# berkeley-hipie/HIPIE

Measured on AMD Instinct MI355X. Metric: images/sec @1024x1024 ViT-H bs=8 (single-image inference hot path: box, class and mask logits), higher is better.
Workload: dtype f16x3 (split-fp16 operands, fp32 accumulate: fp32-class); 1 GPU; BASELINE.json configs[2]: vit_huge, 1024x1024, batch 8 per GPU, 80 class prompts (L=194), detection; global_batch=8, parallelism=dp1, precision_policy=split, launch=eager

## Files before the change

hipie_amd/csrc/gemm.hip:

```cpp
#include "gemm_tile.h"

namespace hipie {

template <typename T>
__global__ __launch_bounds__(256) void to_hl8_kernel(const T* __restrict__ x, f16_t* __restrict__ out, long rows, int K, long ldx, long ldo,
                                                     float scale) {
  const long gid = (long)blockIdx.x * 256 + threadIdx.x;
  const int gpr = K / 8;
  if (gid >= rows * gpr) return;
  const long r = gid / gpr;
  const int g = (int)(gid - r * gpr);
  const T* src = x + r * ldx + 8 * g;
  f16x8 h, l;
#pragma unroll
  for (int e = 0; e < 8; ++e) {
    f16_t hh, ll;
    hl_split((float)src[e] * scale, hh, ll);
    h[e] = hh;
    l[e] = ll;
  }
  f16_t* dst = out + r * ldo + 16 * g;
  *reinterpret_cast<f16x8*>(dst) = h;
  *reinterpret_cast<f16x8*>(dst + 8) = l;
}


constexpr int kTrRows = 128, kTrCols = 64;
__global__ __launch_bounds__(256) void to_hl8_t_kernel(const float* __restrict__ x, f16_t* __restrict__ out, long rows, int C, long ldx,
                                                       long ldo, long rows_p, float scale) {
  __shared__ float tile[kTrRows][kTrCols + 1];
  const long r0 = (long)blockIdx.x * kTrRows;
  const int c0 = blockIdx.y * kTrCols;
  const int tid = threadIdx.x;
  for (int k = tid; k < kTrRows * (kTrCols / 4); k += 256) {
    const int i = k / (kTrCols / 4), j = (k % (kTrCols / 4)) * 4;
    float v[4] = {0.f, 0.f, 0.f, 0.f};
    if (r0 + i < rows) {
      const float* src = x + (r0 + i) * ldx + c0 + j;
      if (c0 + j + 3 < C && (((uintptr_t)src) & 15) == 0) {
        const float4 q = *reinterpret_cast<const float4*>(src);
        v[0] = q.x; v[1] = q.y; v[2] = q.z; v[3] = q.w;
      } else {
        for (int e = 0; e < 4; ++e) v[e] = c0 + j + e < C ? src[e] : 0.f;
      }
    }
    for (int e = 0; e < 4; ++e) tile[i][j + e] = v[e];
  }
  __syncthreads();
  for (int u = tid; u < kTrCols * (kTrRows / 8); u += 256) {
    const int g = u % (kTrRows / 8), c = u / (kTrRows / 8);
    const long m = r0 + 8 * g;
    if (c0 + c >= C || m >= rows_p) continue;
    f16x8 h, l;
#pragma unroll
    for (int e = 0; e < 8; ++e) {
      f16_t hh, ll;
      hl_split(tile[8 * g + e][c] * scale, hh, ll);
      h[e] = hh;
      l[e] = ll;
    }
    f16_t* dst = out + (long)(c0 + c) * ldo + 2 * m;
    *reinterpret_cast<f16x8*>(dst) = h;
    *reinterpret_cast<f16x8*>(dst + 8) = l;
  }
}

}

using namespace hipie;

namespace hipie {
int launch_gemm_k256(const void* X, long ldx_b, int x_f32, const void* W, long ldw_b, const float* bias, float* out, long ldo, int M, int N,
                     hipStream_t st);
}

static int gemm_impl(const void* A, int64_t lda, const void* W, int64_t ldw, const float* bias, const float* resid, int64_t ldr,
                     void* out, int64_t ldo, const int32_t* out_row, const int32_t* a_row, int64_t a_rows, int M, int N, int K, int in_fmt,
                     int out_fmt, int act, float alpha, float oscale, void* stream) {
  HIPIE_REQUIRE(A && W && out, "gemm: null pointer");
  HIPIE_REQUIRE(in_fmt == HIPIE_F16 || in_fmt == HIPIE_HL8 || in_fmt == HIPIE_F32, "gemm: operand format %d (HIPIE_F16 | HIPIE_HL8 | HIPIE_F32)",
                in_fmt);
  HIPIE_REQUIRE(out_fmt == HIPIE_F32 || out_fmt == HIPIE_F16 || out_fmt == HIPIE_HL8, "gemm: output format %d", out_fmt);
  HIPIE_REQUIRE(act >= 0 && act <= 3, "gemm: activation %d (0 none, 1 gelu, 2 relu, 3 quick-gelu)", act);
  HIPIE_REQUIRE(M > 0 && N > 0 && K > 0 && N % 8 == 0, "gemm: M=%d N=%d K=%d (N must be a multiple of 8)", M, N, K);
  const bool a_f32 = in_fmt == HIPIE_F32;
  const bool split = in_fmt == HIPIE_HL8 || a_f32;
  if (a_f32) lda *= 2;
  const int kq = split ? 32 : 64;
  HIPIE_REQUIRE(K % kq == 0, "gemm: K=%d must be a multiple of %d", K, kq);
  const int epr = split ? 2 * K : K;
  HIPIE_TRY(gm_check_operands("gemm", lda, ldw, epr, 320));
  HIPIE_TRY(gm_check_out("gemm", ldo, out_fmt, N));
  HIPIE_TRY(gm_check_resid("gemm", resid, ldr, N));
  HIPIE_TRY(gm_check_aligned("gemm", {A, W, out, bias, resid}));
  GemmParams p;
  gm_set_operands(p, A, lda, W, ldw, M, N, K, kq);
  p.bias = bias; p.resid = resid; p.ldr = ldr; p.out = (char*)out; p.ldo = ldo; p.out_row = out_row; p.a_row = a_row;
  p.out_fmt = out_fmt; p.act = act; p.alpha = alpha; p.oscale = oscale;
  hipStream_t st = (hipStream_t)stream;
  static const int k256_mode = [] { const char* e = study_env("HIPIE_GEMM_K256"); return e ? atoi(e) : 2; }();
  const bool k256_on = k256_mode == 1 || (k256_mode == 2 && N >= 384);
  if (k256_on && split && K == 256 && out_fmt == HIPIE_F32 && act == 0 && resid == nullptr && out_row == nullptr && a_row == nullptr &&
      alpha == 1.f && oscale == 1.f && N % 32 == 0 && M >= 8192 && ldw * 2 == 1024 && (long)M * p.lda_b < (1L << 32))
    return launch_gemm_k256(A, p.lda_b, a_f32 ? 1 : 0, W, p.ldw_b, bias, (float*)out, ldo, M, N, st);
  const bool wide = (N % 320 == 0);
  static const int small_on = [] { const char* e = study_env("HIPIE_GEMM_SMALL"); return e ? atoi(e) : 1; }();
  static const long small_tiles = [] { const char* e = study_env("HIPIE_GEMM_SMALL_MAXTILES"); return e ? atol(e) : 96L; }();
  const bool small_ok = small_on && (long)((M + 255) / 256) * ((N + (wide ? 319 : 255)) / (wide ? 320 : 256)) < small_tiles;
#ifdef HIPIE_GEMM_VARIANTS
  { const char* e = study_env("HIPIE_GEMM_VARIANT"); const int v = e ? atoi(e) : 0;
    if (split && wide && v == 1) return launch_gemm<320, true, 1>(p, st);
    if (split && wide && v == 3) return launch_gemm<320, true, 3>(p, st); }
  { const char* e = study_env("HIPIE_GEMM_VARIANT"); if (e) p.variant = atoi(e); }
  p.prio_mode = gemm2_prio();
  if (split && gemm2_mode() == 4) {
    const bool w160 = (N % 160 == 0);
    if (a_f32) return w160 ? launch_gemm4<5, 2>(p, st) : launch_gemm4<4, 2>(p, st);
    return w160 ? launch_gemm4<5, 0>(p, st) : launch_gemm4<4, 0>(p, st);
  }
  if (split && gemm2_mode() == 2) {
    const bool w160 = (N % 160 == 0);
    if (a_f32) return w160 ? launch_gemm3<5, 2>(p, st) : launch_gemm3<4, 2>(p, st);
    return w160 ? launch_gemm3<5, 0>(p, st) : launch_gemm3<4, 0>(p, st);
  }
  if (split && gemm2_mode() == 1) {
    const bool w160 = (N % 160 == 0);
    if (a_f32) return w160 ? launch_gemm2<5, 2>(p, st) : launch_gemm2<4, 2>(p, st);
    return w160 ? launch_gemm2<5, 0>(p, st) : launch_gemm2<4, 0>(p, st);
  }
#endif
  if (split && small_ok && a_row == nullptr) return a_f32 ? launch_gemm_small<2>(p, st) : launch_gemm_small<0>(p, st);
  if (a_f32) return wide ? launch_gemm<320, true, 2>(p, st) : launch_gemm<256, true, 2>(p, st);
  if (split) return wide ? launch_gemm<320, true>(p, st) : launch_gemm<256, true>(p, st);
  return wide ? launch_gemm<320, false>(p, st) : launch_gemm<256, false>(p, st);
}

extern "C" int hipie_gemm(const void* A, int64_t lda, const void* W, int64_t ldw, const float* bias, const float* resid, int64_t ldr,
                          void* out, int64_t ldo, const int32_t* out_row, int M, int N, int K, int in_fmt, int out_fmt, int act, float alpha,
                          float oscale, void* stream) {
  return gemm_impl(A, lda, W, ldw, bias, resid, ldr, out, ldo, out_row, nullptr, 0, M, N, K, in_fmt, out_fmt, act, alpha, oscale, stream);
}

extern "C" int hipie_gemm_gather(const void* A, int64_t lda, int64_t a_rows, const int32_t* a_row, const void* W, int64_t ldw, const float* bias,
                                 const float* resid, int64_t ldr, void* out, int64_t ldo, const int32_t* out_row, int M, int N, int K, int in_fmt,
                                 int out_fmt, int act, float alpha, float oscale, void* stream) {
  HIPIE_REQUIRE(a_row != nullptr && a_rows > 0, "gemm_gather: a_row map / operand row count missing");
  HIPIE_REQUIRE(in_fmt == HIPIE_HL8 || in_fmt == HIPIE_F32, "gemm_gather: split operands only (HIPIE_HL8 | HIPIE_F32 rows)");
  HIPIE_REQUIRE((long)a_rows * lda * (in_fmt == HIPIE_F32 ? 4 : 2) < (1L << 32), "gemm_gather: the gathered operand must stay below 4 GiB");
  return gemm_impl(A, lda, W, ldw, bias, resid, ldr, out, ldo, out_row, a_row, a_rows, M, N, K, in_fmt, out_fmt, act, alpha, oscale, stream);
}

extern "C" int hipie_gemm_batched(const void* A, int64_t lda, int64_t a_outer, int64_t a_inner, const void* W, int64_t ldw, int64_t w_outer,
                                  int64_t w_inner, void* out, int64_t ldo, int64_t o_outer, int64_t o_inner, int n_outer, int n_inner, int M,
                                  int N, int K, int out_fmt, float alpha, void* stream) {
  HIPIE_REQUIRE(A && W && out, "gemm_batched: null pointer");
  HIPIE_REQUIRE(out_fmt == HIPIE_F32 || out_fmt == HIPIE_HL8, "gemm_batched: output format %d (HIPIE_F32 | HIPIE_HL8)", out_fmt);
  HIPIE_REQUIRE(M > 0 && N > 0 && K > 0 && N % 8 == 0 && K % 32 == 0, "gemm_batched: M=%d N=%d K=%d (N %% 8, K %% 32)", M, N, K);
  HIPIE_TRY(gm_check_batch_shape("gemm_batched", n_outer, n_inner));
  HIPIE_TRY(gm_check_operands("gemm_batched", lda, ldw, 2 * K, 320));
  HIPIE_TRY(gm_check_out("gemm_batched", ldo, out_fmt, N));
  HIPIE_TRY(gm_check_batch_offsets("gemm_batched", a_outer, a_inner, w_outer, w_inner, o_outer, o_inner));
  HIPIE_TRY(gm_check_aligned("gemm_batched", {A, W, out}));
  GemmParams p;
  gm_set_operands(p, A, lda, W, ldw, M, N, K);
  gm_set_batch(p, n_inner, a_outer, a_inner, w_outer, w_inner, o_outer, o_inner, out_fmt == HIPIE_F32 ? 4 : 2);
  p.out = (char*)out; p.ldo = ldo; p.out_fmt = out_fmt; p.alpha = alpha;
  hipStream_t st = (hipStream_t)stream;
  const int batches = n_outer * n_inner;
#ifdef HIPIE_GEMM_VARIANTS
  if (gemm2_mode() == 1) return (N % 160 == 0) ? launch_gemm2<5, 0>(p, st, batches) : launch_gemm2<4, 0>(p, st, batches);
#endif
  return (N % 320 == 0) ? launch_gemm<320, true>(p, st, batches) : launch_gemm<256, true>(p, st, batches);
}

extern "C" int hipie_gemm_batched_resid(const void* A, int64_t lda, int64_t a_outer, int64_t a_inner, const void* W, int64_t ldw, int64_t w_outer,
                                        int64_t w_inner, const float* bias, const float* resid, int64_t ldr, int64_t r_outer, int64_t r_inner,
                                        float* out, int64_t ldo, int64_t o_outer, int64_t o_inner, int n_outer, int n_inner, int M, int N, int K,
                                        float alpha, void* stream) {
  HIPIE_REQUIRE(A && W && out, "gemm_batched_resid: null pointer");
  HIPIE_REQUIRE(M > 0 && N > 0 && K > 0 && N % 8 == 0 && K % 32 == 0, "gemm_batched_resid: M=%d N=%d K=%d (N %% 8, K %% 32)", M, N, K);
  HIPIE_TRY(gm_check_batch_shape("gemm_batched_resid", n_outer, n_inner));
  HIPIE_TRY(gm_check_operands("gemm_batched_resid", lda, ldw, 2 * K, 320));
  HIPIE_TRY(gm_check_out("gemm_batched_resid", ldo, HIPIE_F32, N));
  HIPIE_REQUIRE(resid == nullptr || (ldr >= N && ldr % 4 == 0 && ((r_outer | r_inner) % 4) == 0), "gemm_batched_resid: residual strides %ld / %ld / %ld",
                (long)ldr, (long)r_outer, (long)r_inner);
  HIPIE_TRY(gm_check_batch_offsets("gemm_batched_resid", a_outer, a_inner, w_outer, w_inner, o_outer, o_inner));
  HIPIE_TRY(gm_check_aligned("gemm_batched_resid", {A, W, out, bias, resid}));
  GemmParams p;
  gm_set_operands(p, A, lda, W, ldw, M, N, K);
  gm_set_batch(p, n_inner, a_outer, a_inner, w_outer, w_inner, o_outer, o_inner, 4);
  p.out = (char*)out; p.ldo = ldo; p.alpha = alpha;
  p.bias = bias; p.resid = resid; p.ldr = ldr; p.r_bo = r_outer; p.r_bi = r_inner;
  return (N % 320 == 0) ? launch_gemm<320, true>(p, (hipStream_t)stream, n_outer * n_inner) : launch_gemm<256, true>(p, (hipStream_t)stream, n_outer * n_inner);
}

extern "C" int hipie_gemm_batched_softmax(const void* A, int64_t lda, int64_t a_outer, int64_t a_inner, const void* W, int64_t ldw, int64_t w_outer,
                                          int64_t w_inner, void* out, int64_t ldo, int64_t o_outer, int64_t o_inner, int n_outer, int n_inner,
                                          int M, int N, int K, const unsigned char* mask, int L, float clamp, float alpha, void* stream) {
  HIPIE_REQUIRE(A && W && out, "gemm_batched_softmax: null pointer");
  HIPIE_REQUIRE(M > 0 && N > 0 && N <= 256 && N % 8 == 0 && K > 0 && K % 32 == 0 && L > 0 && L <= N,
                "gemm_batched_softmax: M=%d N=%d K=%d L=%d (N <= 256: the row must fit one column tile)", M, N, K, L);
  HIPIE_TRY(gm_check_batch_shape("gemm_batched_softmax", n_outer, n_inner));
  HIPIE_TRY(gm_check_operands("gemm_batched_softmax", lda, ldw, 2 * K, 320));
  HIPIE_TRY(gm_check_out("gemm_batched_softmax", ldo, HIPIE_HL8, N));
  HIPIE_TRY(gm_check_batch_offsets("gemm_batched_softmax", a_outer, a_inner, w_outer, w_inner, o_outer, o_inner));
  HIPIE_TRY(gm_check_aligned("gemm_batched_softmax", {A, W, out}));
  GemmParams p;
  gm_set_operands(p, A, lda, W, ldw, M, N, K);
  gm_set_batch(p, n_inner, a_outer, a_inner, w_outer, w_inner, o_outer, o_inner, 2);
  p.out = (char*)out; p.ldo = ldo; p.out_fmt = HIPIE_HL8; p.alpha = alpha;
  p.softmax = 1; p.sm_L = L; p.sm_clamp = clamp; p.sm_mask = mask;
  return launch_gemm<256, true>(p, (hipStream_t)stream, n_outer * n_inner);
}

extern "C" int hipie_conv3x3_split(const void* x, int64_t ldx, const void* w, const float* bias, void* out, int64_t ldo, int64_t rows, int Wp,
                                   int C, int N, int in_fmt, int out_fmt, int act, void* stream) {
  HIPIE_REQUIRE(x && w && out, "conv3x3_split: null pointer");
  HIPIE_REQUIRE(in_fmt == HIPIE_HL8 || in_fmt == HIPIE_F32, "conv3x3_split: input format %d (HIPIE_HL8 | HIPIE_F32 rows)", in_fmt);
  HIPIE_REQUIRE(out_fmt == HIPIE_F32 || out_fmt == HIPIE_HL8, "conv3x3_split: output format %d (HIPIE_F32 | HIPIE_HL8)", out_fmt);
  HIPIE_REQUIRE(act >= 0 && act <= 2, "conv3x3_split: activation %d", act);
  HIPIE_REQUIRE(rows > 0 && rows < (1L << 31) && Wp >= 3 && C > 0 && C % 32 == 0 && N > 0 && N % 8 == 0, "conv3x3_split: rows=%ld Wp=%d C=%d N=%d",
                (long)rows, Wp, C, N);
  if (in_fmt == HIPIE_F32) ldx *= 2;
  HIPIE_REQUIRE(ldx >= 2 * C && ldx % 8 == 0, "conv3x3_split: input row stride %ld", (long)ldx);
  HIPIE_REQUIRE((long)(256 + Wp + 2) * ldx * 2 < (1L << 31), "conv3x3_split: row stride too large");
  HIPIE_TRY(gm_check_out("conv3x3_split", ldo, out_fmt, N));
  HIPIE_TRY(gm_check_aligned("conv3x3_split", {x, w, out, bias}));
  GemmParams p;
  gm_set_operands(p, x, ldx, w, (long)2 * 9 * C, (int)rows, N, 9 * C);
  p.bias = bias; p.out = (char*)out; p.ldo = ldo; p.out_fmt = out_fmt; p.act = act;
  p.conv_kpt = C / 32; p.conv_wp = Wp;
  hipStream_t st = (hipStream_t)stream;
  const bool wide = (N % 320 == 0);
  if (in_fmt == HIPIE_F32) return wide ? launch_gemm<320, true, 2>(p, st) : launch_gemm<256, true, 2>(p, st);
  return wide ? launch_gemm<320, true>(p, st) : launch_gemm<256, true>(p, st);
}

extern "C" int hipie_to_hl8(const void* x, int64_t ldx, void* out, int64_t ldo, int64_t rows, int K, int x_dtype, float scale, void* stream) {
  HIPIE_REQUIRE(x && out && rows > 0 && K > 0 && K % 8 == 0, "to_hl8: rows=%ld K=%d (K must be a multiple of 8)", (long)rows, K);
  HIPIE_REQUIRE(ldx >= K && ldo >= 2 * K && ldo % 8 == 0, "to_hl8: row strides %ld / %ld", (long)ldx, (long)ldo);
  const long n = rows * (K / 8);
  const dim3 grid((unsigned)((n + 255) / 256));
  hipStream_t st = (hipStream_t)stream;
  switch (x_dtype) {
    case HIPIE_F32: hipLaunchKernelGGL(to_hl8_kernel<float>, grid, dim3(256), 0, st, (const float*)x, (f16_t*)out, rows, K, ldx, ldo, scale); break;
    case HIPIE_F16: hipLaunchKernelGGL(to_hl8_kernel<f16_t>, grid, dim3(256), 0, st, (const f16_t*)x, (f16_t*)out, rows, K, ldx, ldo, scale); break;
    default: return set_err(HIPIE_EINVAL, "to_hl8: dtype %d", x_dtype);
  }
  return check_launch("to_hl8");
}

extern "C" int hipie_to_hl8_t(const void* x, int64_t ldx, void* out, int64_t ldo, int64_t rows, int C, int64_t rows_p, float scale, void* stream) {
  HIPIE_REQUIRE(x && out && rows > 0 && C > 0, "to_hl8_t: rows=%ld C=%d", (long)rows, C);
  HIPIE_REQUIRE(rows_p >= rows && rows_p % 8 == 0 && ldx >= C && ldo >= 2 * rows_p && ldo % 8 == 0, "to_hl8_t: rows_p=%ld (>= rows, multiple of 8), strides %ld / %ld",
                (long)rows_p, (long)ldx, (long)ldo);
  HIPIE_REQUIRE(((uintptr_t)out % 16) == 0, "to_hl8_t: output must be 16-byte aligned");
  const long tiles_r = (rows_p + kTrRows - 1) / kTrRows, tiles_c = (C + kTrCols - 1) / kTrCols;
  HIPIE_REQUIRE(tiles_c <= 65535, "to_hl8_t: C=%d too wide", C);
  hipLaunchKernelGGL(to_hl8_t_kernel, dim3((unsigned)tiles_r, (unsigned)tiles_c), dim3(256), 0, (hipStream_t)stream, (const float*)x, (f16_t*)out,
                     (long)rows, C, (long)ldx, (long)ldo, (long)rows_p, scale);
  return check_launch("to_hl8_t");
}
```

hipie_amd/csrc/gemm_tile.h:

```cpp
#pragma once
#include <stdlib.h>

#include <initializer_list>

#include "common.h"
#include "gelu.h"
#include "mfma.h"
#include "wave.h"

namespace hipie {

struct GemmParams {
  const char* A = nullptr; const char* W = nullptr; const float* bias = nullptr; const float* resid = nullptr; char* out = nullptr;
  const int32_t* out_row = nullptr;
  const int32_t* a_row = nullptr;
  long lda_b = 0, ldw_b = 0;
  long ldr = 0, ldo = 0;
  int M = 0, N = 0, K = 0;
  int nkt = 0;
  int tiles_m = 0, tiles_n = 0;
  int group_m = 0;
  int out_fmt = HIPIE_F32, act = 0;
  float alpha = 1.f, oscale = 1.f;
  int nbi = 1;
  long a_bo = 0, a_bi = 0, w_bo = 0, w_bi = 0, o_bo = 0, o_bi = 0;
  int conv_kpt = 0, conv_wp = 0;
  int softmax = 0, sm_L = 0;
  float sm_clamp = 0.f;
  const unsigned char* sm_mask = nullptr;
  const float* sm_bias = nullptr;
  long r_bo = 0, r_bi = 0;
  const float* ln_g = nullptr; const float* ln_b = nullptr; float ln_eps = 0.f;
  char* out2 = nullptr; long ldo2 = 0;
  int variant = 0;
  int prio_mode = 0;
};

__device__ __forceinline__ unsigned int gm_pack2(float a, float b) {
  typedef _Float16 h2 __attribute__((ext_vector_type(2)));
  h2 v;
  v[0] = (f16_t)a;
  v[1] = (f16_t)b;
  return __builtin_bit_cast(unsigned int, v);
}

__device__ __forceinline__ unsigned int gm_pack2h(f16_t a, f16_t b) {
  typedef _Float16 h2 __attribute__((ext_vector_type(2)));
  h2 v;
  v[0] = a;
  v[1] = b;
  return __builtin_bit_cast(unsigned int, v);
}


typedef _Float16 gm_h2 __attribute__((ext_vector_type(2)));
__device__ __forceinline__ void gm_split2(float x0, float x1, unsigned int& H, unsigned int& L) {
  x0 = __builtin_amdgcn_fmed3f(x0, -65504.f, 65504.f);
  x1 = __builtin_amdgcn_fmed3f(x1, -65504.f, 65504.f);
  hl_split2(x0, x1, H, L);
}

template <int NG>
__device__ __forceinline__ void gm_epi_vals(const float (&x)[NG][4], const int G0, const float4* rq, const float* sb, const long m, const bool mok,
                                            const int nb, const int hi, const GemmParams& p, const bool has_res) {
  typedef unsigned int u32x2 __attribute__((ext_vector_type(2)));
  typedef unsigned int u32x4 __attribute__((ext_vector_type(4)));
  const float alpha = p.alpha, osc = p.oscale;
  const int act = p.act, ofmt = p.out_fmt;
  float v[NG][4];
#pragma unroll
  for (int g = 0; g < NG; ++g) {
    const float4 b4 = *reinterpret_cast<const float4*>(sb + 8 * (G0 + g) + 4 * hi);
    v[g][0] = x[g][0] * alpha + b4.x;
    v[g][1] = x[g][1] * alpha + b4.y;
    v[g][2] = x[g][2] * alpha + b4.z;
    v[g][3] = x[g][3] * alpha + b4.w;
  }
  if (act == 1) {
#pragma unroll
    for (int g = 0; g < NG; ++g)
#pragma unroll
      for (int e = 0; e < 4; ++e) v[g][e] = gm_gelu(v[g][e]);
  } else if (act == 2) {
#pragma unroll
    for (int g = 0; g < NG; ++g)
#pragma unroll
      for (int e = 0; e < 4; ++e) v[g][e] = fmaxf(v[g][e], 0.f);
  } else if (act == 3) {
#pragma unroll
    for (int g = 0; g < NG; ++g)
#pragma unroll
      for (int e = 0; e < 4; ++e) v[g][e] = v[g][e] / (1.f + expf(-1.702f * v[g][e]));
  }
  if (has_res) {
#pragma unroll
    for (int g = 0; g < NG; ++g) { v[g][0] += rq[g].x; v[g][1] += rq[g].y; v[g][2] += rq[g].z; v[g][3] += rq[g].w; }
  }
  if (osc != 1.f) {
#pragma unroll
    for (int g = 0; g < NG; ++g)
#pragma unroll
      for (int e = 0; e < 4; ++e) v[g][e] *= osc;
  }
  if (ofmt == HIPIE_F16) {
#pragma unroll
    for (int g = 0; g < NG; g += 2) {
      const u32x2 s0 = __builtin_amdgcn_permlane32_swap(gm_pack2(v[g][0], v[g][1]), gm_pack2(v[g + 1][0], v[g + 1][1]), false, false);
      const u32x2 s1 = __builtin_amdgcn_permlane32_swap(gm_pack2(v[g][2], v[g][3]), gm_pack2(v[g + 1][2], v[g + 1][3]), false, false);
      const int n = nb + 8 * (G0 + g + hi);
      if (mok && n < p.N) *reinterpret_cast<u32x4*>(reinterpret_cast<f16_t*>(p.out) + m * p.ldo + n) = (u32x4){s0[0], s1[0], s0[1], s1[1]};
    }
  } else {
    u32x4 piece[NG];
    if (ofmt == HIPIE_F32) {
#pragma unroll
      for (int g = 0; g < NG; ++g)
        piece[g] = (u32x4){__builtin_bit_cast(unsigned int, v[g][0]), __builtin_bit_cast(unsigned int, v[g][1]),
                           __builtin_bit_cast(unsigned int, v[g][2]), __builtin_bit_cast(unsigned int, v[g][3])};
    } else {
#pragma unroll
      for (int g = 0; g < NG; ++g) {
        unsigned int H0, L0, H1, L1;
        gm_split2(v[g][0], v[g][1], H0, L0);
        gm_split2(v[g][2], v[g][3], H1, L1);
#if defined(__HIP_DEVICE_COMPILE__) && !defined(HIPIE_NO_FMA_MIX)
        asm volatile("s_nop 1" : "+v"(H0), "+v"(L0), "+v"(H1), "+v"(L1));
#endif
        const u32x2 s0 = __builtin_amdgcn_permlane32_swap(H0, L0, false, false);
        const u32x2 s1 = __builtin_amdgcn_permlane32_swap(H1, L1, false, false);
        piece[g] = (u32x4){s0[0], s1[0], s0[1], s1[1]};
      }
    }
    const long rowb = (m * p.ldo) * (ofmt == HIPIE_F32 ? 4 : 2) + (long)nb * 4 + 16 * hi;
#pragma unroll
    for (int g = 0; g < NG; ++g)
      if (mok && nb + 8 * (G0 + g) < p.N) *reinterpret_cast<u32x4*>(p.out + rowb + 32 * (G0 + g)) = piece[g];
  }
}

template <int G0, int NG>
__device__ __forceinline__ void gm_epi_quads(const f32x16& a, const float4* rq, const float* sb, const long m, const bool mok, const int nb,
                                             const int hi, const GemmParams& p, const bool has_res) {
  float x[NG][4];
#pragma unroll
  for (int g = 0; g < NG; ++g)
#pragma unroll
    for (int e = 0; e < 4; ++e) x[g][e] = a[4 * (G0 + g) + e];
  gm_epi_vals<NG>(x, G0, rq, sb, m, mok, nb, hi, p, has_res);
}

template <int BN, bool SPLIT, int VAR>
__global__ __launch_bounds__(512, 2) void gemm_kernel(const GemmParams pin) {
  GemmParams p = pin;
  int vtile = -1;
  if (VAR == 8) {
    const int nblk = p.tiles_m * p.tiles_n * p.nbi;
    const int id = blockIdx.x, xcd = id & 7, j = id >> 3;
    const int q = nblk >> 3, r = nblk & 7;
    const int v = (xcd < r ? xcd * (q + 1) : r * (q + 1) + (xcd - r) * q) + j;
    const int bo = blockIdx.y, bi = v % p.nbi;
    vtile = v / p.nbi;
    p.A += bo * p.a_bo + bi * p.a_bi;
    p.W += bo * p.w_bo + bi * p.w_bi;
    p.out += bo * p.o_bo + bi * p.o_bi;
    if (p.sm_mask != nullptr) p.sm_mask += (long)bo * p.sm_L;
    if (p.sm_bias != nullptr) p.sm_bias += ((long)bo * p.nbi + bi) * p.N;
  } else if (gridDim.y > 1) {
    const int bo = blockIdx.y / p.nbi, bi = blockIdx.y - bo * p.nbi;
    p.A += bo * p.a_bo + bi * p.a_bi;
    p.W += bo * p.w_bo + bi * p.w_bi;
    p.out += bo * p.o_bo + bi * p.o_bi;
    if (p.sm_mask != nullptr) p.sm_mask += (long)bo * p.sm_L;
    if (p.sm_bias != nullptr) p.sm_bias += (long)blockIdx.y * p.N;
    if (p.resid != nullptr) p.resid += bo * p.r_bo + bi * p.r_bi;
  }
  constexpr int BM = 256;
  constexpr int ROWS = BM + BN;
  constexpr int STAGE = ROWS * 128;
  constexpr int NI = ROWS / 64;
  constexpr int NJ = BN / 64;
  constexpr int KS = SPLIT ? 2 : 4;
  constexpr int SUB = KS * NJ;
  constexpr bool AF32 = VAR == 2 || VAR == 6;
  constexpr bool LNE = VAR == 4 || VAR == 6;
  typedef Mfma32<f16_t>::frag frag;

  extern __shared__ __attribute__((aligned(128))) char smem[];

  const int tid = threadIdx.x, lane = tid & 63;
  const int wave = __builtin_amdgcn_readfirstlane(tid >> 6);
  const int wm = wave & 3, wn = wave >> 2;
  const int li = lane & 31, hi = lane >> 5;

  int tm, tn;
  {
    const int nblk = p.tiles_m * p.tiles_n;
    const int id = blockIdx.x, xcd = id & 7, j = id >> 3;
    const int q = nblk >> 3, r = nblk & 7;
    const int v = (VAR == 8) ? vtile : (xcd < r ? xcd * (q + 1) : r * (q + 1) + (xcd - r) * q) + j;
    if (p.group_m > 1) {
      const int gsz = p.group_m * p.tiles_n;
      const int g = v / gsz, w = v - g * gsz;
      const int rows = min(p.group_m, p.tiles_m - g * p.group_m);
      tn = w / rows;
      tm = g * p.group_m + (w - tn * rows);
    } else {
      tm = v / p.tiles_n;
      tn = v - tm * p.tiles_n;
    }
  }
  const int m0 = tm * BM, n0 = tn * BN;

  unsigned int dvoff[NI];
  {
    const int rl = lane >> 3, cp = lane & 7;
#pragma unroll
    for (int i = 0; i < NI; ++i) {
      const int r = 8 * (8 * i + wave) + rl;
      const int c = cp ^ ((r >> 1) & 7);
      if (r < BM) {
        const int mr = min(r, p.M - 1 - m0);
        dvoff[i] = p.a_row != nullptr ? (unsigned int)((long)p.a_row[m0 + mr] * p.lda_b + 16 * c) : (unsigned int)((long)mr * p.lda_b + 16 * c);
      } else dvoff[i] = (unsigned int)((long)min(r - BM, p.N - 1 - n0) * p.ldw_b + 16 * c);
    }
  }
  const char* abase = p.a_row != nullptr ? p.A : p.A + (long)m0 * p.lda_b;
  const char* wbase = p.W + (long)n0 * p.ldw_b;
  const unsigned int lds0 = (unsigned int)reinterpret_cast<uintptr_t>((__attribute__((address_space(3))) char*)smem);

  auto dma = [&](const int i, const int kt, const int stage) {
    const bool isa = (8 * (8 * i + wave)) < BM;
    long ko = (long)kt * 128;
    if (isa && p.conv_kpt) {
      const int tap = kt / p.conv_kpt, r = kt - tap * p.conv_kpt, dy = tap / 3;
      ko = ((long)(dy - 1) * p.conv_wp + (tap - 3 * dy - 1)) * p.lda_b + (long)r * 128;
    }
    const char* sb = (isa ? abase : wbase) + ko;
    dma16(sb, dvoff[i], __builtin_amdgcn_readfirstlane(lds0 + (unsigned int)(stage * STAGE + 1024 * (8 * i + wave))));
  };

  const int swz = (li >> 1) & 7;
  const char* xrow = smem + (wm * 64 + li) * 128;
  const char* wrow = smem + (BM + wn * (BN / 2) + li) * 128;
  auto choff = [&](const int ks, const int lo) -> int { return 16 * ((SPLIT ? (2 * (2 * ks + hi) + lo) : (2 * ks + hi)) ^ swz); };

  f32x16 acc[NJ][2];
#pragma unroll
  for (int j = 0; j < NJ; ++j)
#pragma unroll
    for (int t = 0; t < 2; ++t)
#pragma unroll
      for (int r = 0; r < 16; ++r) acc[j][t][r] = 0.f;

#ifdef HIPIE_GEMM_VARIANTS
  const int nkt = (VAR == 3) ? 0 : p.nkt;
  if (VAR != 3)
#else
  const int nkt = p.nkt;
#endif
  {
#pragma unroll
    for (int i = 0; i < NI; ++i) dma(i, 0, 0);
  }
  __builtin_amdgcn_s_waitcnt(vmcnt(0));
  __syncthreads();

  for (int kt = 0; kt < nkt; ++kt) {
    const int st = kt & 1;
    const bool more = kt + 1 < nkt;
    const char* xs = xrow + st * STAGE;
    const char* ws = wrow + st * STAGE;
    frag xa[2][2][2];
    frag wa[2][2];
    auto load_x = [&](const int ks) {
#pragma unroll
      for (int t = 0; t < 2; ++t) {
        xa[ks & 1][0][t] = *reinterpret_cast<const frag*>(xs + t * 4096 + choff(ks, 0));
        if (SPLIT) xa[ks & 1][1][t] = *reinterpret_cast<const frag*>(xs + t * 4096 + choff(ks, 1));
      }
    };
    auto load_w = [&](const int s) {
      const int ks = s / NJ, j = s % NJ;
      wa[s & 1][0] = *reinterpret_cast<const frag*>(ws + j * 4096 + choff(ks, 0));
      if (SPLIT) wa[s & 1][1] = *reinterpret_cast<const frag*>(ws + j * 4096 + choff(ks, 1));
    };
    load_x(0);
    load_w(0);
    constexpr int DMA_BY = SPLIT ? 4 : 6;
    constexpr int PER = (NI + DMA_BY - 1) / DMA_BY;
    frag cx[2][2];
#pragma unroll
    for (int s = 0; s < SUB; ++s) {
      const int ks = s / NJ, j = s % NJ;
      if (s + 1 < SUB) {
        if ((s + 1) % NJ == 0) load_x(ks + 1);
        load_w(s + 1);
      }
      if (AF32 && j == 0) {
#pragma unroll
        for (int t = 0; t < 2; ++t) {
          const f32x4 a = __builtin_bit_cast(f32x4, xa[ks & 1][0][t]), b = __builtin_bit_cast(f32x4, xa[ks & 1][1][t]);
#pragma unroll
          for (int e = 0; e < 4; ++e) {
            f16_t hh, ll;
            hl_split(a[e], hh, ll);
            cx[0][t][e] = hh; cx[1][t][e] = ll;
            hl_split(b[e], hh, ll);
            cx[0][t][4 + e] = hh; cx[1][t][4 + e] = ll;
          }
        }
      }
      const frag wh = wa[s & 1][0];
      const frag xh0 = AF32 ? cx[0][0] : xa[ks & 1][0][0], xh1 = AF32 ? cx[0][1] : xa[ks & 1][0][1];
      if (SPLIT) {
        const frag wl = wa[s & 1][1];
        const frag xl0 = AF32 ? cx[1][0] : xa[ks & 1][1][0], xl1 = AF32 ? cx[1][1] : xa[ks & 1][1][1];
        acc[j][0] = Mfma32<f16_t>::mma(wl, xh0, acc[j][0]);
        acc[j][1] = Mfma32<f16_t>::mma(wl, xh1, acc[j][1]);
        acc[j][0] = Mfma32<f16_t>::mma(wh, xl0, acc[j][0]);
        acc[j][1] = Mfma32<f16_t>::mma(wh, xl1, acc[j][1]);
      }
      acc[j][0] = Mfma32<f16_t>::mma(wh, xh0, acc[j][0]);
      acc[j][1] = Mfma32<f16_t>::mma(wh, xh1, acc[j][1]);
      if (more) {
#pragma unroll
        for (int i = s * PER; i < (s + 1) * PER && i < NI; ++i) dma(i, kt + 1, st ^ 1);
      }
    }
    __builtin_amdgcn_s_waitcnt(vmcnt(0));
    __syncthreads();
  }

  bool has_res = p.resid != nullptr;
#ifdef HIPIE_GEMM_VARIANTS
  if (VAR == 1 && p.alpha != 12345.f) return;
#endif
  const int act = p.act, ofmt = p.out_fmt;
  const float alpha = p.alpha, osc = p.oscale;
  float* sbias = reinterpret_cast<float*>(smem);
  if (tid < BN) sbias[tid] = (p.bias != nullptr && n0 + tid < p.N) ? p.bias[n0 + tid] : 0.f;
  if (SPLIT && LNE && BN == 256) {
    float* lg = sbias + 256;
    float* lb = lg + 256;
    float* red = lb + 256;
    if (tid < 256) { lg[tid] = p.ln_g[tid]; lb[tid] = p.ln_b[tid]; }
    __syncthreads();
    float su[2] = {0.f, 0.f};
    f32x4 rr[2][4];
    auto ln_res = [&](const int blk, f32x4 (&dst)[4]) {
      const int t = blk / NJ, j = blk % NJ;
      const int m = min(m0 + wm * 64 + t * 32 + li, p.M - 1);
#pragma unroll
      for (int g = 0; g < 4; ++g) {
        const int n = wn * (BN / 2) + j * 32 + 8 * g + 4 * hi;
        dst[g] = *reinterpret_cast<const f32x4*>(p.resid + (long)m * p.ldr + n);
      }
    };
    ln_res(0, rr[0]);
#pragma unroll
    for (int blk = 0; blk < 2 * NJ; ++blk) {
      const int t = blk / NJ, j = blk % NJ;
      if (blk + 1 < 2 * NJ) ln_res(blk + 1, rr[(blk + 1) & 1]);
#pragma unroll
      for (int g = 0; g < 4; ++g) {
        const int n = wn * (BN / 2) + j * 32 + 8 * g + 4 * hi;
        const f32x4 b4 = *reinterpret_cast<const f32x4*>(sbias + n);
#pragma unroll
        for (int e = 0; e < 4; ++e) {
          float x = acc[j][t][4 * g + e] * p.alpha + b4[e];
          x += rr[blk & 1][g][e];
          acc[j][t][4 * g + e] = x;
          su[t] += x;
        }
      }
#if defined(__HIP_DEVICE_COMPILE__)
      __builtin_amdgcn_sched_barrier(0);
#endif
    }
#pragma unroll
    for (int t = 0; t < 2; ++t) {
      su[t] += __shfl_xor(su[t], 32);
      if (hi == 0) red[wn * 256 + wm * 64 + t * 32 + li] = su[t];
    }
    __syncthreads();
    float mean[2], sq[2];
#pragma unroll
    for (int t = 0; t < 2; ++t) {
      mean[t] = (su[t] + red[(wn ^ 1) * 256 + wm * 64 + t * 32 + li]) / 256.f;
      float q = 0.f;
#pragma unroll
      for (int j = 0; j < NJ; ++j)
#pragma unroll
        for (int r = 0; r < 16; ++r) { const float d = acc[j][t][r] - mean[t]; q += d * d; }
      sq[t] = q + __shfl_xor(q, 32);
    }
    __syncthreads();
#pragma unroll
    for (int t = 0; t < 2; ++t)
      if (hi == 0) red[wn * 256 + wm * 64 + t * 32 + li] = sq[t];
    __syncthreads();
    float rstd[2];
#pragma unroll
    for (int t = 0; t < 2; ++t) rstd[t] = rsqrtf((sq[t] + red[(wn ^ 1) * 256 + wm * 64 + t * 32 + li]) / 256.f + p.ln_eps);
#pragma unroll
    for (int j = 0; j < NJ; ++j) {
#pragma unroll
      for (int t = 0; t < 2; ++t)
#pragma unroll
        for (int g = 0; g < 4; ++g) {
          const int n = wn * (BN / 2) + j * 32 + 8 * g + 4 * hi;
          const f32x4 g4 = *reinterpret_cast<const f32x4*>(lg + n), b4 = *reinterpret_cast<const f32x4*>(lb + n);
#pragma unroll
          for (int e = 0; e < 4; ++e) acc[j][t][4 * g + e] = (acc[j][t][4 * g + e] - mean[t]) * rstd[t] * g4[e] + b4[e];
        }
#if defined(__HIP_DEVICE_COMPILE__)
      __builtin_amdgcn_sched_barrier(0);
#endif
    }
    __syncthreads();
    if (tid < BN) sbias[tid] = 0.f;
    p.alpha = 1.f; p.act = 0; p.oscale = 1.f; p.out_fmt = HIPIE_F32;
    has_res = false;
  }
  if (SPLIT && (VAR == 0 || VAR == 8) && BN == 256 && p.softmax) {
    float* kb = sbias + 256;
    float* red = kb + 256;
    float* cb = red + 512;
    if (tid < 256) kb[tid] = (tid < p.sm_L && (p.sm_mask == nullptr || p.sm_mask[tid] != 0)) ? 0.f : -INFINITY;
    if (VAR == 8 && tid < 256) cb[tid] = (p.sm_bias != nullptr && tid < p.N) ? p.sm_bias[tid] : 0.f;
    __syncthreads();
    const float cl = p.sm_clamp;
    float mx[2] = {-INFINITY, -INFINITY};
#pragma unroll
    for (int t = 0; t < 2; ++t)
#pragma unroll
      for (int j = 0; j < NJ; ++j)
#pragma unroll
        for (int g = 0; g < 4; ++g) {
          const f32x4 k4 = *reinterpret_cast<const f32x4*>(kb + wn * (BN / 2) + j * 32 + 8 * g + 4 * hi);
          f32x4 c4 = {0.f, 0.f, 0.f, 0.f};
          if (VAR == 8) c4 = *reinterpret_cast<const f32x4*>(cb + wn * (BN / 2) + j * 32 + 8 * g + 4 * hi);
#pragma unroll
          for (int e = 0; e < 4; ++e) {
            float x = acc[j][t][4 * g + e] * p.alpha;
            if (VAR == 8) x += c4[e];
            if (cl > 0.f) x = __builtin_amdgcn_fmed3f(x, -cl, cl);
            x += k4[e];
            acc[j][t][4 * g + e] = x;
            mx[t] = fmaxf(mx[t], x);
          }
        }
#pragma unroll
    for (int t = 0; t < 2; ++t) {
      mx[t] = fmaxf(mx[t], __shfl_xor(mx[t], 32));
      if (hi == 0) red[wn * 256 + wm * 64 + t * 32 + li] = mx[t];
    }
    __syncthreads();
    float sm[2];
#pragma unroll
    for (int t = 0; t < 2; ++t) {
      const float m = fmaxf(mx[t], red[(wn ^ 1) * 256 + wm * 64 + t * 32 + li]);
      const float m2 = (m == -INFINITY) ? 0.f : m * 1.4426950408889634f;
      float su = 0.f;
#pragma unroll
      for (int j = 0; j < NJ; ++j)
#pragma unroll
        for (int r = 0; r < 16; ++r) {
          const float pv = __builtin_amdgcn_exp2f(acc[j][t][r] * 1.4426950408889634f - m2);
          acc[j][t][r] = pv;
          su += pv;
        }
      sm[t] = su + __shfl_xor(su, 32);
    }
    __syncthreads();
#pragma unroll
    for (int t = 0; t < 2; ++t)
      if (hi == 0) red[wn * 256 + wm * 64 + t * 32 + li] = sm[t];
    __syncthreads();
#pragma unroll
    for (int t = 0; t < 2; ++t) {
      const float tot = sm[t] + red[(wn ^ 1) * 256 + wm * 64 + t * 32 + li];
      const float inv = tot > 0.f ? 1.f / tot : 0.f;
#pragma unroll
      for (int j = 0; j < NJ; ++j)
#pragma unroll
        for (int r = 0; r < 16; ++r) acc[j][t][r] *= inv;
    }
    p.alpha = 1.f;
  }
  __syncthreads();
  float4 rq[2][4];
  long orow[2];
#pragma unroll
  for (int t = 0; t < 2; ++t) {
    const int m = m0 + wm * 64 + t * 32 + li;
    orow[t] = (m < p.M) ? (p.out_row != nullptr ? (long)p.out_row[m] : (long)m) : -1;
  }
  auto load_res = [&](const int t, const int j, float4 (&dst)[4]) {
#pragma unroll
    for (int g = 0; g < 4; ++g) {
      const int n = n0 + wn * (BN / 2) + j * 32 + 8 * g + 4 * hi;
      dst[g] = (has_res && orow[t] >= 0 && n < p.N) ? *reinterpret_cast<const float4*>(p.resid + orow[t] * p.ldr + n) : make_float4(0.f, 0.f, 0.f, 0.f);
    }
  };
  const int passes = (LNE && p.out2 != nullptr) ? 2 : 1;
#pragma unroll
  for (int pass = 0; pass < 2; ++pass) {
    if (pass >= passes) break;
    if (pass == 1) { p.out = p.out2; p.ldo = p.ldo2; p.out_fmt = HIPIE_HL8; }
    load_res(0, 0, rq[0]);
#pragma unroll
    for (int t = 0; t < 2; ++t) {
      const long m = orow[t];
      const bool mok = m >= 0;
#pragma unroll
      for (int j = 0; j < NJ; ++j) {
        const int blk = t * NJ + j;
        if (blk + 1 < 2 * NJ) load_res((blk + 1) / NJ, (blk + 1) % NJ, rq[(blk + 1) & 1]);
        const int nb = n0 + wn * (BN / 2) + j * 32;
        gm_epi_quads<0, 4>(acc[j][t], rq[blk & 1], sbias + (nb - n0), m, mok, nb, hi, p, has_res);
#if defined(__HIP_DEVICE_COMPILE__)
        if (LNE) __builtin_amdgcn_sched_barrier(0);
#endif
      }
    }
  }
}



template <int VAR>
__global__ __launch_bounds__(256, 2) void gemm_small_kernel(const GemmParams p) {
  constexpr int BM = 64, BN = 128, ROWS = BM + BN, STAGE = ROWS * 128, NI = ROWS / 32;
  typedef Mfma32<f16_t>::frag frag;
  extern __shared__ __attribute__((aligned(128))) char smem[];

  const int tid = threadIdx.x, lane = tid & 63;
  const int wave = __builtin_amdgcn_readfirstlane(tid >> 6);
  const int li = lane & 31, hi = lane >> 5;
  const int tm = blockIdx.x / p.tiles_n, tn = blockIdx.x - tm * p.tiles_n;
  const int m0 = tm * BM, n0 = tn * BN;

  unsigned int dvoff[NI];
  {
    const int rl = lane >> 3, cp = lane & 7;
#pragma unroll
    for (int i = 0; i < NI; ++i) {
      const int r = 8 * (4 * i + wave) + rl;
      const int c = cp ^ ((r >> 1) & 7);
      if (r < BM) dvoff[i] = (unsigned int)((long)min(r, p.M - 1 - m0) * p.lda_b + 16 * c);
      else dvoff[i] = (unsigned int)((long)min(r - BM, p.N - 1 - n0) * p.ldw_b + 16 * c);
    }
  }
  const char* abase = p.A + (long)m0 * p.lda_b;
  const char* wbase = p.W + (long)n0 * p.ldw_b;
  const unsigned int lds0 = (unsigned int)reinterpret_cast<uintptr_t>((__attribute__((address_space(3))) char*)smem);
  auto dma_stage = [&](const int kt, const int slot) {
#pragma unroll
    for (int i = 0; i < NI; ++i) {
      const bool isa = (8 * (4 * i + wave)) < BM;
      dma16((isa ? abase : wbase) + (long)kt * 128, dvoff[i],
               __builtin_amdgcn_readfirstlane(lds0 + (unsigned int)(slot * STAGE + 1024 * (4 * i + wave))));
    }
  };

  const int swz = (li >> 1) & 7;
  const char* xrow = smem + li * 128;
  const char* wrow = smem + (BM + wave * 32 + li) * 128;
  auto choff = [&](const int ks, const int lo) -> int { return 16 * ((2 * (2 * ks + hi) + lo) ^ swz); };

  f32x16 acc[2];
#pragma unroll
  for (int t = 0; t < 2; ++t)
#pragma unroll
    for (int r = 0; r < 16; ++r) acc[t][r] = 0.f;

  const int nkt = p.nkt;
  dma_stage(0, 0);
  if (nkt > 1) dma_stage(1, 1);
  int slot = 0;
  for (int kt = 0; kt < nkt; ++kt) {
    if (kt + 1 < nkt) __builtin_amdgcn_s_waitcnt(vmcnt(NI));
    else __builtin_amdgcn_s_waitcnt(vmcnt(0));
    __syncthreads();
    if (kt + 2 < nkt) dma_stage(kt + 2, slot == 0 ? 2 : slot - 1);
    const char* xs = xrow + slot * STAGE;
    const char* ws = wrow + slot * STAGE;
#pragma unroll
    for (int ks = 0; ks < 2; ++ks) {
      frag xh[2], xl[2];
#pragma unroll
      for (int t = 0; t < 2; ++t) {
        xh[t] = *reinterpret_cast<const frag*>(xs + t * 4096 + choff(ks, 0));
        xl[t] = *reinterpret_cast<const frag*>(xs + t * 4096 + choff(ks, 1));
      }
      const frag wh = *reinterpret_cast<const frag*>(ws + choff(ks, 0));
      const frag wl = *reinterpret_cast<const frag*>(ws + choff(ks, 1));
      if (VAR == 2) {
#pragma unroll
        for (int t = 0; t < 2; ++t) {
          const f32x4 a = __builtin_bit_cast(f32x4, xh[t]), b = __builtin_bit_cast(f32x4, xl[t]);
#pragma unroll
          for (int e = 0; e < 4; ++e) {
            f16_t hh, ll;
            hl_split(a[e], hh, ll);
            xh[t][e] = hh; xl[t][e] = ll;
            hl_split(b[e], hh, ll);
            xh[t][4 + e] = hh; xl[t][4 + e] = ll;
          }
        }
      }
#pragma unroll
      for (int t = 0; t < 2; ++t) {
        acc[t] = Mfma32<f16_t>::mma(wl, xh[t], acc[t]);
        acc[t] = Mfma32<f16_t>::mma(wh, xl[t], acc[t]);
        acc[t] = Mfma32<f16_t>::mma(wh, xh[t], acc[t]);
      }
    }
    slot = slot == 2 ? 0 : slot + 1;
  }

  const bool has_res = p.resid != nullptr;
  __syncthreads();
  float* sbias = reinterpret_cast<float*>(smem);
  if (tid < BN) sbias[tid] = (p.bias != nullptr && n0 + tid < p.N) ? p.bias[n0 + tid] : 0.f;
  __syncthreads();
  const int nb = n0 + wave * 32;
#pragma unroll
  for (int t = 0; t < 2; ++t) {
    const int mm = m0 + t * 32 + li;
    const long m = (mm < p.M) ? (p.out_row != nullptr ? (long)p.out_row[mm] : (long)mm) : -1;
    float4 rq[4];
#pragma unroll
    for (int g = 0; g < 4; ++g) {
      const int n = nb + 8 * g + 4 * hi;
      rq[g] = (has_res && m >= 0 && n < p.N) ? *reinterpret_cast<const float4*>(p.resid + m * p.ldr + n) : make_float4(0.f, 0.f, 0.f, 0.f);
    }
    gm_epi_quads<0, 4>(acc[t], rq, sbias + wave * 32, m, m >= 0, nb, hi, p, has_res);
  }
}

template <int VAR>
static int launch_gemm_small(GemmParams& p, hipStream_t st) {
  constexpr size_t lds = (size_t)3 * (64 + 128) * 128;
  p.tiles_m = (p.M + 63) / 64;
  p.tiles_n = (p.N + 127) / 128;
  auto kern = gemm_small_kernel<VAR>;
  static LdsLimit limit;
  limit.raise((const void*)kern, lds);
  hipLaunchKernelGGL(kern, dim3((unsigned)(p.tiles_m * p.tiles_n)), dim3(256), lds, st, p);
  return check_launch("gemm_small");
}

#ifdef HIPIE_GEMM_VARIANTS
#include "../../tools/ubench/gemm_overlap_study.h"
#endif

template <int BN, bool SPLIT, int VAR = 0>
static int launch_gemm(GemmParams& p, hipStream_t st, int batches = 1) {
  constexpr size_t lds = (size_t)2 * (256 + BN) * 128;
  p.tiles_m = (p.M + 255) / 256;
  p.tiles_n = (p.N + BN - 1) / BN;
  p.group_m = p.tiles_n > 4 ? 8 : 0;
  auto kern = gemm_kernel<BN, SPLIT, VAR>;
  static LdsLimit limit;
  limit.raise((const void*)kern, lds);
  if (VAR == 8)
    hipLaunchKernelGGL(kern, dim3((unsigned)(p.tiles_m * p.tiles_n * p.nbi), (unsigned)(batches / p.nbi)), dim3(512), lds, st, p);
  else
    hipLaunchKernelGGL(kern, dim3((unsigned)(p.tiles_m * p.tiles_n), (unsigned)batches), dim3(512), lds, st, p);
  return check_launch("gemm");
}

static inline void gm_set_operands(GemmParams& p, const void* A, long lda, const void* W, long ldw, int M, int N, int K, int kq = 32) {
  p.A = (const char*)A; p.W = (const char*)W;
  p.lda_b = lda * 2; p.ldw_b = ldw * 2;
  p.M = M; p.N = N; p.K = K; p.nkt = K / kq;
}

static inline void gm_set_batch(GemmParams& p, int n_inner, long a_outer, long a_inner, long w_outer, long w_inner, long o_outer, long o_inner,
                                long osz) {
  p.nbi = n_inner;
  p.a_bo = a_outer * 2; p.a_bi = a_inner * 2; p.w_bo = w_outer * 2; p.w_bi = w_inner * 2; p.o_bo = o_outer * osz; p.o_bi = o_inner * osz;
}

static inline int gm_check_operands(const char* who, long lda, long ldw, int epr, int bn) {
  if (!(lda >= epr && ldw >= epr && lda % 8 == 0 && ldw % 8 == 0))
    return set_err(HIPIE_EINVAL, "%s: operand row strides %ld / %ld (>= %d, multiples of 8)", who, lda, ldw, epr);
  if (!(256 * lda * 2 < (1L << 31) && bn * ldw * 2 < (1L << 31))) return set_err(HIPIE_EINVAL, "%s: row stride too large", who);
  return 0;
}

static inline int gm_check_out(const char* who, long ldo, int out_fmt, int N) {
  const int opr = out_fmt == HIPIE_HL8 ? 2 * N : N;
  if (!(ldo >= opr && ldo % 4 == 0)) return set_err(HIPIE_EINVAL, "%s: output row stride %ld (>= %d)", who, ldo, opr);
  return 0;
}

static inline int gm_check_resid(const char* who, const float* resid, long ldr, int N) {
  if (!(resid == nullptr || (ldr >= N && ldr % 4 == 0))) return set_err(HIPIE_EINVAL, "%s: residual row stride %ld", who, ldr);
  return 0;
}

static inline int gm_check_batch_shape(const char* who, int n_outer, int n_inner) {
  if (!(n_outer > 0 && n_inner > 0 && (long)n_outer * n_inner <= 65535)) return set_err(HIPIE_EINVAL, "%s: %d x %d problems", who, n_outer, n_inner);
  return 0;
}

static inline int gm_check_batch_offsets(const char* who, long a_outer, long a_inner, long w_outer, long w_inner, long o_outer, long o_inner) {
  if (!(((a_outer | a_inner | w_outer | w_inner) % 8) == 0 && ((o_outer | o_inner) % 4) == 0))
    return set_err(HIPIE_EINVAL, "%s: batch offsets must keep 16-byte alignment", who);
  return 0;
}

static inline int gm_check_aligned(const char* who, std::initializer_list<const void*> ptrs) {
  for (const void* q : ptrs)
    if ((uintptr_t)q % 16 != 0) return set_err(HIPIE_EINVAL, "%s: pointers must be 16-byte aligned", who);
  return 0;
}

}
```

hipie_amd/csrc/mfma.h:

```cpp
#pragma once
#include "common.h"

namespace hipie {

__device__ __forceinline__ int crow(int r, int hi) { return (r & 3) + 8 * (r >> 2) + 4 * hi; }

template <typename T> struct Mfma32;
template <> struct Mfma32<bf16_t> {
  typedef bf16x8 frag;
  typedef bf16x4 half_frag;
  static __device__ __forceinline__ f32x16 mma(frag a, frag b, f32x16 c) {
    return __builtin_amdgcn_mfma_f32_32x32x16_bf16(a, b, c, 0, 0, 0);
  }
  static __device__ __forceinline__ half_frag tr_read(const bf16_t* lds_ptr) {
    return __builtin_bit_cast(bf16x4, __builtin_amdgcn_ds_read_tr16_b64_v4i16((__attribute__((address_space(3))) i16x4*)lds_ptr));
  }
};
template <> struct Mfma32<f16_t> {
  typedef f16x8 frag;
  typedef f16x4 half_frag;
  static __device__ __forceinline__ f32x16 mma(frag a, frag b, f32x16 c) {
    return __builtin_amdgcn_mfma_f32_32x32x16_f16(a, b, c, 0, 0, 0);
  }
  static __device__ __forceinline__ half_frag tr_read(const f16_t* lds_ptr) {
    return __builtin_bit_cast(f16x4, __builtin_amdgcn_ds_read_tr16_b64_v4i16((__attribute__((address_space(3))) i16x4*)lds_ptr));
  }
};

}
```

Baseline: 41.77 images/sec.

## Add 16x16x32 MFMA path for wide split-fp16 GEMM tiles

Adds a second main-loop body for the wide (BN=320) split-precision GEMM that uses 16x16x32 f16 MFMA instructions instead of 32x32x16. It brings a new LDS swizzle, a fragment register rotation for W, interleaved DMA prefetch, and a new epilogue that uses permlane16_swap to pack outputs. The path is on by default unless HIPIE_GEMM_MFMA selects otherwise. The aim is better MFMA issue rate and latency hiding for the three-product hi/lo scheme, at the cost of more LDS reads per FLOP and a different register footprint.

```diff
diff --git a/hipie_amd/csrc/gemm.hip b/hipie_amd/csrc/gemm.hip
--- a/hipie_amd/csrc/gemm.hip
+++ b/hipie_amd/csrc/gemm.hip
@@ -74,6 +74,11 @@
                      hipStream_t st);
 }
 
+static inline bool gemm_mfma16() {
+  const char* e = study_env("HIPIE_GEMM_MFMA");
+  return e ? atoi(e) == 16 : true;
+}
+
 static int gemm_impl(const void* A, int64_t lda, const void* W, int64_t ldw, const float* bias, const float* resid, int64_t ldr,
                      void* out, int64_t ldo, const int32_t* out_row, const int32_t* a_row, int64_t a_rows, int M, int N, int K, int in_fmt,
                      int out_fmt, int act, float alpha, float oscale, void* stream) {
@@ -130,6 +135,7 @@
   }
 #endif
   if (split && small_ok && a_row == nullptr) return a_f32 ? launch_gemm_small<2>(p, st) : launch_gemm_small<0>(p, st);
+  if (split && wide && gemm_mfma16()) return a_f32 ? launch_gemm<320, true, 2, 16>(p, st) : launch_gemm<320, true, 0, 16>(p, st);
   if (a_f32) return wide ? launch_gemm<320, true, 2>(p, st) : launch_gemm<256, true, 2>(p, st);
   if (split) return wide ? launch_gemm<320, true>(p, st) : launch_gemm<256, true>(p, st);
   return wide ? launch_gemm<320, false>(p, st) : launch_gemm<256, false>(p, st);
diff --git a/hipie_amd/csrc/gemm_tile.h b/hipie_amd/csrc/gemm_tile.h
--- a/hipie_amd/csrc/gemm_tile.h
+++ b/hipie_amd/csrc/gemm_tile.h
@@ -149,8 +149,203 @@
   gm_epi_vals<NG>(x, G0, rq, sb, m, mok, nb, hi, p, has_res);
 }
 
-template <int BN, bool SPLIT, int VAR>
+__device__ __forceinline__ constexpr int gm_swz16(const int r) { return ((r >> 1) & 3) | (((((r & 15) + 4) >> 3) & 1) << 2); }
+
+__device__ __forceinline__ void gm_epi_vals16(const float (&x)[2][4], const float4* rq, const float* sb, const long m, const bool mok, const int nb,
+                                              const int g, const GemmParams& p, const bool has_res) {
+  typedef unsigned int u32x2 __attribute__((ext_vector_type(2)));
+  typedef unsigned int u32x4 __attribute__((ext_vector_type(4)));
+  const float alpha = p.alpha, osc = p.oscale;
+  const int act = p.act, ofmt = p.out_fmt;
+  float v[2][4];
+#pragma unroll
+  for (int i = 0; i < 2; ++i) {
+    const float4 b4 = *reinterpret_cast<const float4*>(sb + 16 * i + 4 * g);
+    v[i][0] = x[i][0] * alpha + b4.x;
+    v[i][1] = x[i][1] * alpha + b4.y;
+    v[i][2] = x[i][2] * alpha + b4.z;
+    v[i][3] = x[i][3] * alpha + b4.w;
+  }
+  if (act == 1) {
+#pragma unroll
+    for (int i = 0; i < 2; ++i)
+#pragma unroll
+      for (int e = 0; e < 4; ++e) v[i][e] = gm_gelu(v[i][e]);
+  } else if (act == 2) {
+#pragma unroll
+    for (int i = 0; i < 2; ++i)
+#pragma unroll
+      for (int e = 0; e < 4; ++e) v[i][e] = fmaxf(v[i][e], 0.f);
+  } else if (act == 3) {
+#pragma unroll
+    for (int i = 0; i < 2; ++i)
+#pragma unroll
+      for (int e = 0; e < 4; ++e) v[i][e] = v[i][e] / (1.f + expf(-1.702f * v[i][e]));
+  }
+  if (has_res) {
+#pragma unroll
+    for (int i = 0; i < 2; ++i) { v[i][0] += rq[i].x; v[i][1] += rq[i].y; v[i][2] += rq[i].z; v[i][3] += rq[i].w; }
+  }
+  if (osc != 1.f) {
+#pragma unroll
+    for (int i = 0; i < 2; ++i)
+#pragma unroll
+      for (int e = 0; e < 4; ++e) v[i][e] *= osc;
+  }
+  if (ofmt == HIPIE_F16) {
+    const u32x2 s0 = __builtin_amdgcn_permlane16_swap(gm_pack2(v[0][0], v[0][1]), gm_pack2(v[1][0], v[1][1]), false, false);
+    const u32x2 s1 = __builtin_amdgcn_permlane16_swap(gm_pack2(v[0][2], v[0][3]), gm_pack2(v[1][2], v[1][3]), false, false);
+    const int n = nb + 16 * (g & 1) + 8 * (g >> 1);
+    if (mok && n < p.N) *reinterpret_cast<u32x4*>(reinterpret_cast<f16_t*>(p.out) + m * p.ldo + n) = (u32x4){s0[0], s1[0], s0[1], s1[1]};
+  } else {
+    u32x4 piece[2];
+    if (ofmt == HIPIE_F32) {
+#pragma unroll
+      for (int i = 0; i < 2; ++i)
+        piece[i] = (u32x4){__builtin_bit_cast(unsigned int, v[i][0]), __builtin_bit_cast(unsigned int, v[i][1]),
+                           __builtin_bit_cast(unsigned int, v[i][2]), __builtin_bit_cast(unsigned int, v[i][3])};
+    } else {
+#pragma unroll
+      for (int i = 0; i < 2; ++i) {
+        unsigned int H0, L0, H1, L1;
+        gm_split2(v[i][0], v[i][1], H0, L0);
+        gm_split2(v[i][2], v[i][3], H1, L1);
+#if defined(__HIP_DEVICE_COMPILE__) && !defined(HIPIE_NO_FMA_MIX)
+        asm volatile("s_nop 1" : "+v"(H0), "+v"(L0), "+v"(H1), "+v"(L1));
+#endif
+        const u32x2 s0 = __builtin_amdgcn_permlane16_swap(H0, L0, false, false);
+        const u32x2 s1 = __builtin_amdgcn_permlane16_swap(H1, L1, false, false);
+        piece[i] = (u32x4){s0[0], s1[0], s0[1], s1[1]};
+      }
+    }
+    const long rowb = (m * p.ldo) * (ofmt == HIPIE_F32 ? 4 : 2) + (long)nb * 4 + 16 * g;
+#pragma unroll
+    for (int i = 0; i < 2; ++i)
+      if (mok && nb + 16 * i < p.N) *reinterpret_cast<u32x4*>(p.out + rowb + 64 * i) = piece[i];
+  }
+}
+
+template <int BN, bool AF32, typename Dma>
+__device__ __forceinline__ void gm_body16(const GemmParams& p, char* smem, const Dma& dma, const int m0, const int n0, const int wm, const int wn,
+                                          const int tid) {
+  constexpr int BM = 256, ROWS = BM + BN, STAGE = ROWS * 128, NI = ROWS / 64;
+  constexpr int NT = 4;
+  constexpr int NF = BN / 32;
+  typedef Mfma16<f16_t>::frag frag;
+  const int lane = tid & 63, c = lane & 15, g = lane >> 4;
+
+  const int swz = gm_swz16(c);
+  const char* xrow = smem + (wm * 64 + c) * 128;
+  const char* wrow = smem + (BM + wn * (BN / 2) + c) * 128;
+  const int ch[2] = {16 * ((2 * g) ^ swz), 16 * ((2 * g + 1) ^ swz)};
+
+  f32x4 acc[NF][NT];
+#pragma unroll
+  for (int j = 0; j < NF; ++j)
+#pragma unroll
+    for (int t = 0; t < NT; ++t) acc[j][t] = (f32x4){0.f, 0.f, 0.f, 0.f};
+
+  const int nkt = p.nkt;
+#pragma unroll
+  for (int i = 0; i < NI; ++i) dma(i, 0, 0);
+  __builtin_amdgcn_s_waitcnt(vmcnt(0));
+  __syncthreads();
+
+  for (int kt = 0; kt < nkt; ++kt) {
+    const int st = kt & 1;
+    const bool more = kt + 1 < nkt;
+    const char* xs = xrow + st * STAGE;
+    const char* ws = wrow + st * STAGE;
+    frag xa[2][NT];
+    frag wa[3][2];
+    auto load_w = [&](const int j) {
+      wa[j % 3][0] = *reinterpret_cast<const frag*>(ws + j * 2048 + ch[0]);
+      wa[j % 3][1] = *reinterpret_cast<const frag*>(ws + j * 2048 + ch[1]);
+    };
+#pragma unroll
+    for (int t = 0; t < NT; ++t) {
+      xa[0][t] = *reinterpret_cast<const frag*>(xs + t * 2048 + ch[0]);
+      xa[1][t] = *reinterpret_cast<const frag*>(xs + t * 2048 + ch[1]);
+    }
+    load_w(0);
+    load_w(1);
+    if (AF32) {
+#pragma unroll
+      for (int t = 0; t < NT; ++t) {
+        const f32x4 a = __builtin_bit_cast(f32x4, xa[0][t]), b = __builtin_bit_cast(f32x4, xa[1][t]);
+#pragma unroll
+        for (int e = 0; e < 4; ++e) {
+          f16_t hh, ll;
+          hl_split(a[e], hh, ll);
+          xa[0][t][e] = hh; xa[1][t][e] = ll;
+          hl_split(b[e], hh, ll);
+          xa[0][t][4 + e] = hh; xa[1][t][4 + e] = ll;
+        }
+      }
+    }
+    constexpr int DMA_BY = 4;
+    constexpr int PER = (NI + DMA_BY - 1) / DMA_BY;
+#pragma unroll
+    for (int j = 0; j < NF; ++j) {
+      if (j + 2 < NF) load_w(j + 2);
+      const frag wh = wa[j % 3][0], wl = wa[j % 3][1];
+#pragma unroll
+      for (int t = 0; t < NT; ++t) acc[j][t] = Mfma16<f16_t>::mma(wl, xa[0][t], acc[j][t]);
+#pragma unroll
+      for (int t = 0; t < NT; ++t) acc[j][t] = Mfma16<f16_t>::mma(wh, xa[1][t], acc[j][t]);
+#pragma unroll
+      for (int t = 0; t < NT; ++t) acc[j][t] = Mfma16<f16_t>::mma(wh, xa[0][t], acc[j][t]);
+      if (more) {
+#pragma unroll
+        for (int i = j * PER; i < (j + 1) * PER && i < NI; ++i) dma(i, kt + 1, st ^ 1);
+      }
+    }
+    __builtin_amdgcn_s_waitcnt(vmcnt(0));
+    __syncthreads();
+  }
+
+  const bool has_res = p.resid != nullptr;
+  float* sbias = reinterpret_cast<float*>(smem);
+  if (tid < BN) sbias[tid] = (p.bias != nullptr && n0 + tid < p.N) ? p.bias[n0 + tid] : 0.f;
+  __syncthreads();
+  long orow[NT];
+#pragma unroll
+  for (int t = 0; t < NT; ++t) {
+    const int m = m0 + wm * 64 + t * 16 + c;
+    orow[t] = (m < p.M) ? (p.out_row != nullptr ? (long)p.out_row[m] : (long)m) : -1;
+  }
+  float4 rq[2][2];
+  auto load_res = [&](const int blk, float4 (&dst)[2]) {
+    const int t = blk / (NF / 2), jp = blk % (NF / 2);
+#pragma unroll
+    for (int i = 0; i < 2; ++i) {
+      const int n = n0 + wn * (BN / 2) + jp * 32 + 16 * i + 4 * g;
+      dst[i] = (has_res && orow[t] >= 0 && n < p.N) ? *reinterpret_cast<const float4*>(p.resid + orow[t] * p.ldr + n) : make_float4(0.f, 0.f, 0.f, 0.f);
+    }
+  };
+  load_res(0, rq[0]);
+#pragma unroll
+  for (int t = 0; t < NT; ++t) {
+    const long m = orow[t];
+#pragma unroll
+    for (int jp = 0; jp < NF / 2; ++jp) {
+      const int blk = t * (NF / 2) + jp;
+      if (blk + 1 < NT * (NF / 2)) load_res(blk + 1, rq[(blk + 1) & 1]);
+      const int nb = n0 + wn * (BN / 2) + jp * 32;
+      float x[2][4];
+#pragma unroll
+      for (int i = 0; i < 2; ++i)
+#pragma unroll
+        for (int e = 0; e < 4; ++e) x[i][e] = acc[2 * jp + i][t][e];
+      gm_epi_vals16(x, rq[blk & 1], sbias + (nb - n0), m, m >= 0, nb, g, p, has_res);
+    }
+  }
+}
+
+template <int BN, bool SPLIT, int VAR, int MS = 32>
 __global__ __launch_bounds__(512, 2) void gemm_kernel(const GemmParams pin) {
+  static_assert(MS == 32 || (MS == 16 && BN == 320 && SPLIT && (VAR == 0 || VAR == 2)),
+                "the 16x16x32 form exists for the wide split instances (HL8 and fp32 A rows) only");
   GemmParams p = pin;
   int vtile = -1;
   if (VAR == 8) {
@@ -217,7 +412,7 @@
 #pragma unroll
     for (int i = 0; i < NI; ++i) {
       const int r = 8 * (8 * i + wave) + rl;
-      const int c = cp ^ ((r >> 1) & 7);
+      const int c = cp ^ (MS == 16 ? gm_swz16(r) : ((r >> 1) & 7));
       if (r < BM) {
         const int mr = min(r, p.M - 1 - m0);
         dvoff[i] = p.a_row != nullptr ? (unsigned int)((long)p.a_row[m0 + mr] * p.lda_b + 16 * c) : (unsigned int)((long)mr * p.lda_b + 16 * c);
@@ -238,6 +433,11 @@
     const char* sb = (isa ? abase : wbase) + ko;
     dma16(sb, dvoff[i], __builtin_amdgcn_readfirstlane(lds0 + (unsigned int)(stage * STAGE + 1024 * (8 * i + wave))));
   };
+
+  if constexpr (MS == 16) {
+    gm_body16<BN, VAR == 2>(p, smem, dma, m0, n0, wm, wn, tid);
+    return;
+  }
 
   const int swz = (li >> 1) & 7;
   const char* xrow = smem + (wm * 64 + li) * 128;
@@ -656,13 +856,13 @@
 #include "../../tools/ubench/gemm_overlap_study.h"
 #endif
 
-template <int BN, bool SPLIT, int VAR = 0>
+template <int BN, bool SPLIT, int VAR = 0, int MS = 32>
 static int launch_gemm(GemmParams& p, hipStream_t st, int batches = 1) {
   constexpr size_t lds = (size_t)2 * (256 + BN) * 128;
   p.tiles_m = (p.M + 255) / 256;
   p.tiles_n = (p.N + BN - 1) / BN;
   p.group_m = p.tiles_n > 4 ? 8 : 0;
-  auto kern = gemm_kernel<BN, SPLIT, VAR>;
+  auto kern = gemm_kernel<BN, SPLIT, VAR, MS>;
   static LdsLimit limit;
   limit.raise((const void*)kern, lds);
   if (VAR == 8)
diff --git a/hipie_amd/csrc/mfma.h b/hipie_amd/csrc/mfma.h
--- a/hipie_amd/csrc/mfma.h
+++ b/hipie_amd/csrc/mfma.h
@@ -27,4 +27,12 @@
   }
 };
 
+template <typename T> struct Mfma16;
+template <> struct Mfma16<f16_t> {
+  typedef f16x8 frag;
+  static __device__ __forceinline__ f32x4 mma(frag a, frag b, f32x4 c) {
+    return __builtin_amdgcn_mfma_f32_16x16x32_f16(a, b, c, 0, 0, 0);
+  }
+};
+
 }
```

Result: faster. 43.64 images/sec, median of 6 (+4.5%).
